# ingonyama-zk/gnark-icicle

Measured on AMD Instinct MI355X. Metric: BN254 G1 MSM Mpoints/s (2^20 points per GPU, sharded MSM), higher is better.
Workload: dtype u32 limbs (BN254 Fp/Fr Montgomery, integer); 1 GPU; BN254 G1 MSM 2^20 random points/scalars per GPU (BASELINE configs[1]); points_per_gpu=1048576, total_points=1048576, parallelism=msm-shard1

## Files before the change

### gnark-icicle_amd/csrc/curve.hpp

```cpp
#pragma once
#include "field.hpp"

namespace gm {

template <class F>
struct FOps;

template <class P>
struct FOps<Fe<P>> {
  using T = Fe<P>;
  GM_DEV static T zero() { return fe_zero<P>(); }
  GM_DEV static T one() { return fe_one<P>(); }
};
template <class P, int B>
struct FOps<Fe2<P, B>> {
  using T = Fe2<P, B>;
  GM_DEV static T zero() { return {fe_zero<P>(), fe_zero<P>()}; }
  GM_DEV static T one() { return {fe_one<P>(), fe_zero<P>()}; }
};

template <class F>
struct Affine {
  F x, y;
};
template <class F>
struct XYZZ {
  F x, y, zz, zzz;
};

template <class F>
GM_DEV bool aff_is_inf(const Affine<F>& p) {
  return fe_is_zero(p.x) && fe_is_zero(p.y);
}

template <class F>
GM_DEV XYZZ<F> xyzz_inf() {
  XYZZ<F> r;
  r.x = FOps<F>::one();
  r.y = FOps<F>::one();
  r.zz = FOps<F>::zero();
  r.zzz = FOps<F>::zero();
  return r;
}
template <class F>
GM_DEV bool xyzz_is_inf(const XYZZ<F>& p) {
  return fe_is_zero(p.zz);
}

template <class F>
GM_DEV XYZZ<F> xyzz_dbl_aff(const Affine<F>& p) {
  F U = fe_dbl(p.y);
  F V = fe_sqr(U);
  F W = fe_mul(U, V);
  F S = fe_mul(p.x, V);
  F X2 = fe_sqr(p.x);
  F M = fe_add(fe_dbl(X2), X2);
  XYZZ<F> r;
  r.x = fe_sub(fe_sqr(M), fe_dbl(S));
  r.y = fe_sub(fe_mul(M, fe_sub(S, r.x)), fe_mul(W, p.y));
  r.zz = V;
  r.zzz = W;
  return r;
}

template <class F>
GM_DEV void xyzz_add_aff(XYZZ<F>& a, const Affine<F>& p) {
  if (aff_is_inf(p)) return;
  if (xyzz_is_inf(a)) {
    a.x = p.x;
    a.y = p.y;
    a.zz = FOps<F>::one();
    a.zzz = FOps<F>::one();
    return;
  }
  F P = fe_sub(fe_mul(p.x, a.zz), a.x);
  F R = fe_sub(fe_mul(p.y, a.zzz), a.y);
  if (fe_is_zero(P)) {
    if (fe_is_zero(R)) {
      a = xyzz_dbl_aff(p);
    } else {
      a = xyzz_inf<F>();
    }
    return;
  }
  F PP = fe_sqr(P);
  F PPP = fe_mul(P, PP);
  a.zz = fe_mul(a.zz, PP);
  F Q = fe_mul(a.x, PP);
  a.zzz = fe_mul(a.zzz, PPP);
  F X3 = fe_sub(fe_sub(fe_sqr(R), PPP), fe_dbl(Q));
  a.y = fe_sub(fe_mul(R, fe_sub(Q, X3)), fe_mul(a.y, PPP));
  a.x = X3;
}

template <class P, int CH = 0>
GM_DEV void xyzz_add_aff_lz(XYZZ<Fe<P>>& a, const Affine<Fe<P>>& p, bool neg) {
  static_assert(P::BITS + 7 <= RADIX * P::N, "lazy reduction needs R' > 128 p");
  using F = Fe<P>;
  if (aff_is_inf(p)) return;
  if (xyzz_is_inf(a)) {
    a.x = p.x;
    a.y = neg ? fe_neg(p.y) : p.y;
    a.zz = fe_one<P>();
    a.zzz = fe_one<P>();
    return;
  }
  F Pd = fe_sub_lz<8>(fe_mul<P, false, CH>(p.x, a.zz), a.x);
  F R = fe_sub_lz<4>(fe_cneg2p_cf(fe_mul<P, false, CH>(p.y, a.zzz), neg), a.y);
  if (fe_is_zero_lz<10>(Pd)) {
    if (fe_is_zero_lz<6>(R)) {
      Affine<F> q = p;
      if (neg) q.y = fe_neg(p.y);
      a = xyzz_dbl_aff(q);
    } else {
      a = xyzz_inf<F>();
    }
    return;
  }
  F PP = fe_sqr<P, false, CH>(Pd);
  F PPP = fe_mul<P, false, CH>(Pd, PP);
  a.zz = fe_mul<P, false, CH>(a.zz, PP);
  F Q = fe_mul<P, false, CH>(a.x, PP);
  a.zzz = fe_mul<P, false, CH>(a.zzz, PPP);
  F X3 = fe_sub2x_lz<6>(fe_sqr<P, false, CH>(R), PPP, Q);
  if constexpr (P::N <= 10)
    a.y = fe_mul2_redc_u<P, CH>(R, fe_sub_cf<9>(Q, X3), fe_negk_cf<5>(a.y), PPP);
  else
    a.y = fe_mul2_redc_u<P, CH>(R, fe_sub_lz<8>(Q, X3), fe_negk_cf<5>(a.y), PPP);
  a.x = X3;
}
template <class P, int BETA>
GM_DEV void xyzz_add_aff_lz(XYZZ<Fe2<P, BETA>>& a, const Affine<Fe2<P, BETA>>& p) {
  static_assert(P::BITS + 7 <= RADIX * P::N, "lazy reduction needs R' > 128 p");
  using F = Fe2<P, BETA>;
  if (aff_is_inf(p)) return;
  if (xyzz_is_inf(a)) {
    a.x = p.x;
    a.y = p.y;
    a.zz = FOps<F>::one();
    a.zzz = FOps<F>::one();
    return;
  }
  F Pd = fe2_sub_lz<2>(fe2_mul_lz(p.x, a.zz), a.x);
  F R = fe2_sub_lz<2>(fe2_mul_lz(p.y, a.zzz), a.y);
  if (fe_is_zero_lz<4>(Pd.a0) && fe_is_zero_lz<4>(Pd.a1)) {
    if (fe_is_zero_lz<4>(R.a0) && fe_is_zero_lz<4>(R.a1)) {
      a = xyzz_dbl_aff(p);
    } else {
      a = xyzz_inf<F>();
    }
    return;
  }
  F PP = fe2_sqr_lz<4>(Pd);
  F PPP = fe2_mul_lz(Pd, PP);
  a.zz = fe2_mul_lz(a.zz, PP);
  F Q = fe2_mul_lz(a.x, PP);
  a.zzz = fe2_mul_lz(a.zzz, PPP);
  F X3 = fe2_sub_lz<4>(fe2_sub_lz<2>(fe2_sqr_lz<4>(R), PPP), fe2_add_lz(Q, Q));
  fe2_to2p<8>(X3);
  F Y3 = fe2_sub_lz<2>(fe2_mul_lz(R, fe2_sub_lz<2>(Q, X3)), fe2_mul_lz(a.y, PPP));
  fe2_to2p<4>(Y3);
  a.x = X3;
  a.y = Y3;
}
template <class P, int BETA>
GM_DEV XYZZ<Fe2<P, BETA>> xyzz_canon_lz(const XYZZ<Fe2<P, BETA>>& a) {
  auto c = [](const Fe2<P, BETA>& v) { return Fe2<P, BETA>{fe_canon<1>(v.a0), fe_canon<1>(v.a1)}; };
  return {c(a.x), c(a.y), c(a.zz), c(a.zzz)};
}

template <class P>
GM_DEV XYZZ<Fe<P>> xyzz_canon_lz(const XYZZ<Fe<P>>& a) {
  XYZZ<Fe<P>> r;
  r.x = fe_canon<3>(a.x);
  r.y = fe_canon<2>(a.y);
  r.zz = fe_canon<1>(a.zz);
  r.zzz = fe_canon<1>(a.zzz);
  return r;
}

template <class F>
GM_DEV XYZZ<F> xyzz_dbl(const XYZZ<F>& a) {
  F U = fe_dbl(a.y);
  F V = fe_sqr(U);
  F W = fe_mul(U, V);
  F S = fe_mul(a.x, V);
  F X2 = fe_sqr(a.x);
  F M = fe_add(fe_dbl(X2), X2);
  XYZZ<F> r;
  r.x = fe_sub(fe_sqr(M), fe_dbl(S));
  r.y = fe_sub(fe_mul(M, fe_sub(S, r.x)), fe_mul(W, a.y));
  r.zz = fe_mul(V, a.zz);
  r.zzz = fe_mul(W, a.zzz);
  return r;
}

template <class F>
GM_DEV XYZZ<F> xyzz_add(const XYZZ<F>& a, const XYZZ<F>& b) {
  if (xyzz_is_inf(a)) return b;
  if (xyzz_is_inf(b)) return a;
  F U1 = fe_mul(a.x, b.zz);
  F U2 = fe_mul(b.x, a.zz);
  F S1 = fe_mul(a.y, b.zzz);
  F S2 = fe_mul(b.y, a.zzz);
  F P = fe_sub(U2, U1);
  F R = fe_sub(S2, S1);
  if (fe_is_zero(P)) {
    if (fe_is_zero(R)) return xyzz_dbl(a);
    return xyzz_inf<F>();
  }
  F PP = fe_sqr(P);
  F PPP = fe_mul(P, PP);
  F Q = fe_mul(U1, PP);
  XYZZ<F> r;
  r.x = fe_sub(fe_sub(fe_sqr(R), PPP), fe_dbl(Q));
  r.y = fe_sub(fe_mul(R, fe_sub(Q, r.x)), fe_mul(S1, PPP));
  r.zz = fe_mul(fe_mul(a.zz, b.zz), PP);
  r.zzz = fe_mul(fe_mul(a.zzz, b.zzz), PPP);
  return r;
}

template <class P>
GM_DEV XYZZ<Fe<P>> xyzz_canon2(const XYZZ<Fe<P>>& a) {
  return {fe_canon<1>(a.x), fe_canon<1>(a.y), fe_canon<1>(a.zz), fe_canon<1>(a.zzz)};
}

template <class P>
GM_DEV XYZZ<Fe<P>> xyzz_add_lz(const XYZZ<Fe<P>>& a, const XYZZ<Fe<P>>& b) {
  using F = Fe<P>;
  if (xyzz_is_inf(a)) return b;
  if (xyzz_is_inf(b)) return a;
  const F U1 = fe_mul_lz(a.x, b.zz);
  const F U2 = fe_mul_lz(b.x, a.zz);
  const F S1 = fe_mul_lz(a.y, b.zzz);
  const F S2 = fe_mul_lz(b.y, a.zzz);
  const F Pd = fe_sub_lz<2>(U2, U1);
  const F R = fe_sub_lz<2>(S2, S1);
  if (fe_is_zero_lz<4>(Pd)) {
    if (fe_is_zero_lz<4>(R)) return xyzz_dbl(xyzz_canon2(a));
    return xyzz_inf<F>();
  }
  const F PP = fe_sqr_lz(Pd);
  const F PPP = fe_mul_lz(Pd, PP);
  const F Q = fe_mul_lz(U1, PP);
  F X3 = fe_sub_lz<4>(fe_sub_lz<2>(fe_sqr_lz(R), PPP), fe_add_lz(Q, Q));
  fe_to2p<8>(X3);
  const F Y3 = fe_mul2_redc_u(R, fe_sub_lz<2>(Q, X3), fe_negk_cf<3>(S1), PPP);
  XYZZ<F> r;
  r.x = X3;
  r.y = Y3;
  r.zz = fe_mul_lz(fe_mul_lz(a.zz, b.zz), PP);
  r.zzz = fe_mul_lz(fe_mul_lz(a.zzz, b.zzz), PPP);
  return r;
}

template <class F>
GM_DEV Affine<F> load_affine_gnark(const uint32_t* __restrict__ src) {
  Affine<F> r;
  r.x = Coord<F>::load_internal(src);
  r.y = Coord<F>::load_internal(src + Coord<F>::WORDS);
  return r;
}
template <class F>
GM_DEV Affine<F> load_affine_packed(const uint32_t* __restrict__ src) {
  Affine<F> r;
  r.x = Coord<F>::load_packed(src);
  r.y = Coord<F>::load_packed(src + Coord<F>::WORDS);
  return r;
}
template <class F>
GM_DEV void store_affine_packed(uint32_t* __restrict__ dst, const Affine<F>& a) {
  Coord<F>::store_packed(dst, a.x);
  Coord<F>::store_packed(dst + Coord<F>::WORDS, a.y);
}
template <class F>
GM_DEV void store_affine_gnark(uint32_t* __restrict__ dst, const Affine<F>& a) {
  Coord<F>::store_gnark(dst, a.x);
  Coord<F>::store_gnark(dst + Coord<F>::WORDS, a.y);
}

template <class F>
GM_DEV Affine<F> aff_neg(const Affine<F>& p) {
  Affine<F> r;
  r.x = p.x;
  r.y = fe_neg(p.y);
  return r;
}

template <class F>
GM_DEV XYZZ<F> xyzz_mul_small(const XYZZ<F>& a, uint32_t k) {
  XYZZ<F> r = xyzz_inf<F>();
  if (k == 0) return r;
  int top = 31 - __builtin_clz(k);
  r = a;
  for (int b = top - 1; b >= 0; b--) {
    r = xyzz_dbl(r);
    if ((k >> b) & 1) r = xyzz_add(r, a);
  }
  return r;
}

using Bn254Fp2 = Fe2<Bn254Fp, -1>;
using Bls377Fp2 = Fe2<Bls377Fp, -5>;

}
```

### gnark-icicle_amd/csrc/field.hpp

```cpp
#pragma once
#include <hip/hip_runtime.h>
#include <cstdint>
#include "field_constants.hpp"

namespace gm {

#define GM_DEV __device__ __forceinline__
#define GM_HD __host__ __device__ __forceinline__

constexpr int RADIX = 29;
constexpr uint32_t LIMB_MASK = (1u << RADIX) - 1;

#define GM_CONST_ARRAY_FN(FN, N, INIT)       \
  GM_HD static constexpr uint32_t FN(int i) { \
    constexpr uint32_t a[N] = INIT;           \
    return a[i];                              \
  }

#define GM_DEFINE_FIELD(NAME, TAG)                                              \
  struct NAME {                                                                 \
    static constexpr int N = GM_##TAG##_N29;              \
    static constexpr int NG = GM_##TAG##_NG;               \
    static constexpr int BITS = GM_##TAG##_BITS;                                \
    static constexpr uint32_t INV = GM_##TAG##_INV29;                           \
// ... 225 lines not shown
    for (int i = (k - N + 1 > 0 ? k - N + 1 : 0); i <= (k - 1 < N - 1 ? k - 1 : N - 1); i++) {
      acc += (uint64_t)m[i] * P::p(k - i);
      GM_STRICT_STEP(acc, CHAIN);
    }
    if (k < N) {
      m[k] = ((uint32_t)acc * P::INV) & LIMB_MASK;
      acc += (uint64_t)m[k] * P::p(0);
    } else {
      r.v[k - N] = (uint32_t)acc & LIMB_MASK;
    }
    acc >>= RADIX;
  }
  r.v[N - 1] = (uint32_t)acc;
  if constexpr (REDUCE) fe_reduce_once(r);
  return r;
}

template <class P, bool REDUCE = true, int CHAIN = GM_FE_CHAIN>
GM_DEV Fe<P> fe_sqr(const Fe<P>& a) {
  constexpr int N = P::N;
  uint32_t m[N];
  Fe<P> r;
  uint64_t acc = 0;
#pragma unroll
  for (int k = 0; k < 2 * N - 1; k++) {
    if constexpr (CHAIN) {
      if (k) __asm__ volatile("" : "+v"(acc));
    }
    if constexpr (CHAIN >= 2) {
#pragma unroll
      for (int i = (k - N + 1 > 0 ? k - N + 1 : 0); i <= (k < N - 1 ? k : N - 1); i++) {
        const int j = k - i;
        if (i < j) {
          acc += (uint64_t)a.v[i] * (a.v[j] << 1);
          GM_STRICT_STEP(acc, CHAIN);
        }
      }
    } else {
      uint64_t cross = 0;
#pragma unroll
      for (int i = (k - N + 1 > 0 ? k - N + 1 : 0); i <= (k < N - 1 ? k : N - 1); i++) {
        const int j = k - i;
        if (i < j) cross += (uint64_t)a.v[i] * a.v[j];
      }
      acc += cross << 1;
    }
    if ((k & 1) == 0) {
      acc += (uint64_t)a.v[k / 2] * a.v[k / 2];
      GM_STRICT_STEP(acc, CHAIN);
    }
#pragma unroll
    for (int i = (k - N + 1 > 0 ? k - N + 1 : 0); i <= (k - 1 < N - 1 ? k - 1 : N - 1); i++) {
      acc += (uint64_t)m[i] * P::p(k - i);
      GM_STRICT_STEP(acc, CHAIN);
    }
    if (k < N) {
      m[k] = ((uint32_t)acc * P::INV) & LIMB_MASK;
      acc += (uint64_t)m[k] * P::p(0);
    } else {
      r.v[k - N] = (uint32_t)acc & LIMB_MASK;
    }
    acc >>= RADIX;
  }
  r.v[N - 1] = (uint32_t)acc;
  if constexpr (REDUCE) fe_reduce_once(r);
  return r;
}

template <class P, int K>
GM_HD constexpr uint32_t kp_limb(int i) {
  uint64_t carry = 0;
  for (int j = 0; j < P::N; j++) {
    const uint64_t v = (uint64_t)P::p(j) * K + carry;
    if (j == i) return j == P::N - 1 ? (uint32_t)v : (uint32_t)(v & LIMB_MASK);
    carry = v >> RADIX;
  }
  return 0;
}
template <class P>
GM_HD constexpr uint32_t kp_top(int j) {
  uint64_t carry = 0, v = 0;
  for (int i = 0; i < P::N; i++) {
    v = (uint64_t)P::p(i) * (uint64_t)j + carry;
    carry = v >> RADIX;
  }
  return (uint32_t)v;
}
template <class P>
GM_DEV Fe<P> fe_mul_lz(const Fe<P>& a, const Fe<P>& b) { return fe_mul<P, false>(a, b); }
template <class P>
GM_DEV Fe<P> fe_mul_lz_chain(const Fe<P>& a, const Fe<P>& b) { return fe_mul<P, false, true>(a, b); }
template <class P>
GM_DEV Fe<P> fe_sqr_lz(const Fe<P>& a) { return fe_sqr<P, false>(a); }
template <class P, int CHAIN = GM_FE_CHAIN>
GM_DEV Fe<P> fe_mul2_redc_u(const Fe<P>& x1, const Fe<P>& y1, const Fe<P>& x2, const Fe<P>& y2) {
  constexpr int N = P::N;
  static_assert(N <= 14, "unsigned two-product column bound");
  uint32_t m[N];
  Fe<P> r;
  uint64_t acc = 0;
#pragma unroll
  for (int k = 0; k < 2 * N - 1; k++) {
    if constexpr (CHAIN) {
      if (k) __asm__ volatile("" : "+v"(acc));
    }
#pragma unroll
    for (int i = (k - N + 1 > 0 ? k - N + 1 : 0); i <= (k < N - 1 ? k : N - 1); i++) {
      acc += (uint64_t)x1.v[i] * y1.v[k - i];
      GM_STRICT_STEP(acc, CHAIN);
      acc += (uint64_t)x2.v[i] * y2.v[k - i];
      GM_STRICT_STEP(acc, CHAIN);
    }
#pragma unroll
    for (int i = (k - N + 1 > 0 ? k - N + 1 : 0); i <= (k - 1 < N - 1 ? k - 1 : N - 1); i++) {
      acc += (uint64_t)m[i] * P::p(k - i);
      GM_STRICT_STEP(acc, CHAIN);
    }
    if (k < N) {
      m[k] = ((uint32_t)acc * P::INV) & LIMB_MASK;
      acc += (uint64_t)m[k] * P::p(0);
    } else {
      r.v[k - N] = (uint32_t)acc & LIMB_MASK;
    }
    acc >>= RADIX;
  }
  r.v[N - 1] = (uint32_t)acc;
  return r;
}

template <class P>
GM_DEV Fe<P> fe_add_lz(const Fe<P>& a, const Fe<P>& b) {
  Fe<P> r;
  uint32_t c = 0;
#pragma unroll
  for (int i = 0; i < P::N; i++) {
    const uint32_t s = a.v[i] + b.v[i] + c;
    r.v[i] = i == P::N - 1 ? s : (s & LIMB_MASK);
    c = s >> RADIX;
  }
  return r;
}
template <int K, class P>
GM_DEV Fe<P> fe_sub_lz(const Fe<P>& a, const Fe<P>& b) {
  Fe<P> r;
  int32_t c = 0;
#pragma unroll
  for (int i = 0; i < P::N; i++) {
    const int32_t d = (int32_t)(a.v[i] + kp_limb<P, K>(i)) - (int32_t)b.v[i] + c;
    c = d >> RADIX;
    r.v[i] = i == P::N - 1 ? (uint32_t)d : ((uint32_t)d & LIMB_MASK);
  }
  return r;
}
template <int K, class P>
GM_DEV void fe_reduce_k(Fe<P>& a) {
  Fe<P> t;
  int32_t borrow = 0;
#pragma unroll
  for (int i = 0; i < P::N; i++) {
    const int32_t d = (int32_t)a.v[i] - (int32_t)kp_limb<P, K>(i) + borrow;
    borrow = d >> RADIX;
    t.v[i] = (uint32_t)d & LIMB_MASK;
  }
  const bool ge = borrow == 0;
#pragma unroll
  for (int i = 0; i < P::N; i++) a.v[i] = ge ? t.v[i] : a.v[i];
}
template <class P>
GM_HD constexpr uint32_t p2_borrowed_limb(int i) {
  return i == 0 ? kp_limb<P, 2>(0) + (1u << RADIX)
                : (i == P::N - 1 ? kp_limb<P, 2>(i) - 1u : kp_limb<P, 2>(i) + (1u << RADIX) - 1u);
}
template <class P, int K>
GM_HD constexpr uint32_t kp_borrowed_limb(int i) {
  return i == 0 ? kp_limb<P, K>(0) + (1u << RADIX)
                : (i == P::N - 1 ? kp_limb<P, K>(i) - 1u : kp_limb<P, K>(i) + (1u << RADIX) - 1u);
}
template <int K, class P>
GM_DEV Fe<P> fe_negk_cf(const Fe<P>& s) {
  Fe<P> r;
#pragma unroll
  for (int i = 0; i < P::N; i++) r.v[i] = kp_borrowed_limb<P, K>(i) - s.v[i];
  return r;
}
template <int K, class P>
GM_DEV Fe<P> fe_sub_cf(const Fe<P>& a, const Fe<P>& b) {
  static_assert(P::N <= 11, "unnormalised product operand column bound");
  Fe<P> r;
#pragma unroll
  for (int i = 0; i < P::N; i++) r.v[i] = a.v[i] + (kp_borrowed_limb<P, K>(i) - b.v[i]);
  return r;
}
template <class P>
GM_DEV Fe<P> fe_cneg2p_cf(const Fe<P>& s, bool neg) {
  Fe<P> r;
#pragma unroll
  for (int i = 0; i < P::N; i++) r.v[i] = neg ? p2_borrowed_limb<P>(i) - s.v[i] : s.v[i];
  return r;
}
template <int K, class P>
GM_DEV Fe<P> fe_sub2x_lz(const Fe<P>& a, const Fe<P>& b, const Fe<P>& c) {
  Fe<P> r;
  int32_t cy = 0;
#pragma unroll
  for (int i = 0; i < P::N; i++) {
    const int32_t d = (int32_t)(a.v[i] + kp_limb<P, K>(i)) - (int32_t)(b.v[i] + (c.v[i] << 1)) + cy;
    cy = d >> RADIX;
    r.v[i] = i == P::N - 1 ? (uint32_t)d : ((uint32_t)d & LIMB_MASK);
  }
  return r;
}
template <int L, class P>
GM_DEV Fe<P> fe_canon(Fe<P> a) {
  if constexpr (L >= 4) fe_reduce_k<8>(a);
  if constexpr (L >= 3) fe_reduce_k<4>(a);
  if constexpr (L >= 2) fe_reduce_k<2>(a);
  if constexpr (L >= 1) fe_reduce_k<1>(a);
  return a;
}
template <int K, class P>
GM_DEV bool fe_is_zero_lz(const Fe<P>& a) {
  static_assert(K <= 16, "fe_canon<4> covers a < 16p");
  const uint32_t top = a.v[P::N - 1];
  bool hit = false;
#pragma unroll
  for (int j = 0; j < K; j++) hit |= top == kp_top<P>(j);
  if (!hit) return false;
  return fe_is_zero(fe_canon<4>(a));
}

template <class P>
GM_DEV Fe<P> fe_to_internal(const Fe<P>& gnark_form) { return fe_mul(gnark_form, GM_FE_CONST(P, kin)); }
template <class P>
GM_DEV Fe<P> fe_to_gnark(const Fe<P>& internal) { return fe_mul(internal, GM_FE_CONST(P, kout)); }
template <class P>
GM_DEV Fe<P> fe_gnark_to_canonical(const Fe<P>& gnark_form) { return fe_mul(gnark_form, GM_FE_CONST(P, kcan)); }
template <class P>
GM_DEV Fe<P> fe_canonical_to_gnark(const Fe<P>& x) { return fe_mul(x, GM_FE_CONST(P, kgn)); }
template <class P>
GM_DEV Fe<P> fe_to_mont(const Fe<P>& x) { return fe_mul(x, GM_FE_CONST(P, r2)); }
template <class P>
GM_DEV Fe<P> fe_from_mont(const Fe<P>& internal) {
  Fe<P> o = fe_zero<P>();
  o.v[0] = 1;
  return fe_mul(internal, o);
}

template <class P>
GM_DEV Fe<P> fe_inv(const Fe<P>& a) {
  Fe<P> r = fe_one<P>();
  for (int i = P::NG - 1; i >= 0; i--) {
    const uint32_t e = P::pm2(i);
    for (int b = 31; b >= 0; b--) {
      r = fe_sqr(r);
      if ((e >> b) & 1) r = fe_mul(r, a);
    }
  }
  return r;
}

template <class P, int BETA>
struct Fe2 {
  using Base = P;
  Fe<P> a0, a1;
};

template <class P, int BETA>
GM_DEV Fe2<P, BETA> fe_add(const Fe2<P, BETA>& a, const Fe2<P, BETA>& b) {
  return {fe_add(a.a0, b.a0), fe_add(a.a1, b.a1)};
}
template <class P, int BETA>
GM_DEV Fe2<P, BETA> fe_sub(const Fe2<P, BETA>& a, const Fe2<P, BETA>& b) {
  return {fe_sub(a.a0, b.a0), fe_sub(a.a1, b.a1)};
}
template <class P, int BETA>
GM_DEV Fe2<P, BETA> fe_dbl(const Fe2<P, BETA>& a) {
  return {fe_dbl(a.a0), fe_dbl(a.a1)};
}
template <class P, int BETA>
GM_DEV Fe2<P, BETA> fe_neg(const Fe2<P, BETA>& a) {
  return {fe_neg(a.a0), fe_neg(a.a1)};
}
template <class P, int BETA>
GM_DEV bool fe_is_zero(const Fe2<P, BETA>& a) {
  return fe_is_zero(a.a0) && fe_is_zero(a.a1);
}
template <class P, int BETA>
GM_DEV Fe<P> mul_by_beta(const Fe<P>& x) {
  static_assert(BETA == -1 || BETA == -5, "unsupported non-residue");
  if constexpr (BETA == -1) {
    return fe_neg(x);
  } else {
    Fe<P> x2 = fe_dbl(x);
    Fe<P> x4 = fe_dbl(x2);
    return fe_neg(fe_add(x4, x));
  }
}
template <class P, int BETA>
GM_DEV Fe2<P, BETA> fe_mul(const Fe2<P, BETA>& a, const Fe2<P, BETA>& b) {
  Fe<P> v0 = fe_mul(a.a0, b.a0);
  Fe<P> v1 = fe_mul(a.a1, b.a1);
  Fe<P> s = fe_mul(fe_add(a.a0, a.a1), fe_add(b.a0, b.a1));
  Fe2<P, BETA> r;
  r.a0 = fe_add(v0, mul_by_beta<P, BETA>(v1));
  r.a1 = fe_sub(fe_sub(s, v0), v1);
  return r;
// ... 116 lines not shown
```

### gnark-icicle_amd/csrc/msm_impl.hpp

```cpp
#pragma once
#include "curves.hpp"
#include "msm.hpp"
#include "pair_fp2.hpp"
#include "runtime.hpp"

#include <hip/hip_ext.h>

#include <cmath>
#include <cstdlib>
#include <cstring>
#include <type_traits>

namespace gm {

template <class Fr>
GM_DEV uint32_t window_bits(const FeG<Fr>& k, uint32_t bit, uint32_t mask) {
  const uint32_t idx = bit >> 5, sh = bit & 31;
  uint32_t lo = 0, hi = 0;
#pragma unroll
  for (int i = 0; i < Fr::NG; i++) {
    lo = (idx == (uint32_t)i) ? k.w[i] : lo;
    hi = (idx + 1 == (uint32_t)i) ? k.w[i] : hi;
  }
  const uint64_t v = ((uint64_t)hi << 32) | lo;
// ... 192 lines not shown
  static constexpr bool ok = true;
  using U = unsigned __int128;
  GM_DEV static void split(const uint64_t (&k64)[4], U& k1, U& k2, uint32_t& neg2) {
    U q = glv_mulshift<5>(k64, GlvBls377::g);
    const U lam = ((U)GlvBls377::LAM_HI << 64) | GlvBls377::LAM_LO;
    const U klo = ((U)k64[1] << 64) | k64[0];
    U r = klo - q * lam;
    if (r >= lam) {
      r -= lam;
      q += 1;
    }
    k1 = r;
    k2 = q;
    neg2 = 0;
  }
};

template <class C>
__global__ void __launch_bounds__(1024) k_msm_digits_glv(const uint32_t* __restrict__ scalars, DigitGeom g,
                                                         uint32_t n0, uint32_t NC, uint32_t* __restrict__ dig,
                                                         uint32_t* __restrict__ ccount) {
  using Fr = typename C::Fr;
  extern __shared__ uint32_t dg_lds[];
  const uint32_t t = threadIdx.x;
  for (uint32_t q = t; q < NC; q += DG_THREADS) dg_lds[q] = 0;
  __syncthreads();
  const uint32_t base = blockIdx.x * DG_THREADS * DG_PPT;
  for (uint32_t r = 0; r < DG_PPT; r++) {
    const uint32_t i = base + r * DG_THREADS + t;
    if (i >= n0) break;
    const FeG<Fr> k = load_scalar_canonical<Fr>(scalars, i);
    uint64_t k64[4];
#pragma unroll
    for (int j = 0; j < 4; j++) k64[j] = (uint64_t)k.w[2 * j] | ((uint64_t)k.w[2 * j + 1] << 32);
    unsigned __int128 k1, k2;
    uint32_t neg2;
    Glv<C>::split(k64, k1, k2, neg2);
    FeG<Fr> m1, m2;
#pragma unroll
    for (int j = 0; j < Fr::NG; j++) {
      m1.w[j] = j < 4 ? (uint32_t)(k1 >> (32 * j)) : 0u;
      m2.w[j] = j < 4 ? (uint32_t)(k2 >> (32 * j)) : 0u;
    }
    emit_digits<Fr>(m1, 0u, i, g, dig, dg_lds);
    emit_digits<Fr>(m2, neg2, n0 + i, g, dig, dg_lds);
  }
  __syncthreads();
  for (uint32_t q = t; q < NC; q += DG_THREADS)
    if (dg_lds[q]) atomicAdd(&ccount[q], dg_lds[q]);
}

template <class F, bool GLV>
__global__ void __launch_bounds__(256) k_msm_convert_points_lds(const uint32_t* __restrict__ src, size_t n,
                                                                uint32_t* __restrict__ dst) {
  constexpr int PW = 2 * Coord<F>::WORDS;
  constexpr uint32_t Q = PW / 4;
  static_assert(PW % 4 == 0, "points are whole uint4s");
  __shared__ uint4 tile[256 * (Q + 1)];
  const size_t b0 = (size_t)blockIdx.x * 256;
  const uint32_t np = (uint32_t)min((size_t)256, n - b0);
  const uint32_t t = threadIdx.x;
  const uint4* s = reinterpret_cast<const uint4*>(src) + b0 * Q;
  for (uint32_t q = t; q < np * Q; q += 256) tile[(q / Q) * (Q + 1) + q % Q] = s[q];
  __syncthreads();
  uint32_t* mine = reinterpret_cast<uint32_t*>(tile + t * (Q + 1));
  Affine<F> a;
  if (t < np) {
    a = load_affine_gnark<F>(mine);
    store_affine_packed<F>(mine, a);
  }
  __syncthreads();
  uint4* d = reinterpret_cast<uint4*>(dst) + b0 * Q;
  for (uint32_t q = t; q < np * Q; q += 256) d[q] = tile[(q / Q) * (Q + 1) + q % Q];
  if constexpr (GLV) {
    __syncthreads();
    if (t < np) {
      a.x = glv_phi_x(a.x);
      store_affine_packed<F>(mine, a);
    }
    __syncthreads();
    uint4* d2 = reinterpret_cast<uint4*>(dst) + (n + b0) * Q;
    for (uint32_t q = t; q < np * Q; q += 256) d2[q] = tile[(q / Q) * (Q + 1) + q % Q];
  }
}

template <class F>
__global__ void __launch_bounds__(256) k_msm_convert_points(const uint32_t* __restrict__ src, size_t n,
                                                            uint32_t* __restrict__ dst) {
  const size_t i = (size_t)blockIdx.x * blockDim.x + threadIdx.x;
  if (i >= n) return;
  constexpr int PW = 2 * Coord<F>::WORDS;
  store_affine_packed<F>(dst + i * PW, load_affine_gnark<F>(src + i * PW));
}

template <class F>
__global__ void __launch_bounds__(128) k_msm_precompute(uint32_t* __restrict__ pts, size_t n, size_t stride,
                                                        uint32_t c, uint32_t W, uint32_t wn) {
  const size_t i = (size_t)blockIdx.x * blockDim.x + threadIdx.x;
  if (i >= n) return;
  constexpr int PW = 2 * Coord<F>::WORDS;
  const Affine<F> P = load_affine_packed<F>(pts + i * PW);
  Affine<F> zero;
  zero.x = FOps<F>::zero();
  zero.y = FOps<F>::zero();
  if (aff_is_inf(P)) {
    for (uint32_t w = 1; w < W; w++) store_affine_packed<F>(pts + (w * stride + i) * PW, zero);
    return;
  }
  XYZZ<F> acc;
  acc.x = P.x;
  acc.y = P.y;
  acc.zz = FOps<F>::one();
  acc.zzz = FOps<F>::one();
  for (uint32_t w = 1; w < W; w++) {
    const uint32_t cw = (w - 1 >= wn) ? c - 1 : c;
    for (uint32_t k = 0; k < cw; k++) acc = xyzz_dbl(acc);
    Affine<F> r = zero;
    if (!xyzz_is_inf(acc)) {
      const F t = fe_inv(fe_mul(acc.zz, acc.zzz));
      r.x = fe_mul(acc.x, fe_mul(t, acc.zzz));
      r.y = fe_mul(acc.y, fe_mul(t, acc.zz));
    }
    store_affine_packed<F>(pts + (w * stride + i) * PW, r);
  }
}

template <int PW>
struct PackedPt {
  uint32_t w[PW];
};
template <int PW>
GM_DEV PackedPt<PW> load_packed_pt(const uint32_t* __restrict__ src) {
  static_assert(PW % 4 == 0, "packed points are whole 16-byte chunks");
  PackedPt<PW> r;
#pragma unroll
  for (int q = 0; q < PW / 4; q++) {
    const uint4 v = reinterpret_cast<const uint4*>(src)[q];
    r.w[4 * q] = v.x;
    r.w[4 * q + 1] = v.y;
    r.w[4 * q + 2] = v.z;
    r.w[4 * q + 3] = v.w;
  }
  return r;
}

template <class F>
struct LazyAcc {
  static constexpr bool on = false;
  template <bool CH = false>
  GM_DEV static void add(XYZZ<F>& a, Affine<F> p, bool neg) {
    if (neg) p.y = fe_neg(p.y);
    xyzz_add_aff(a, p);
  }
  GM_DEV static XYZZ<F> canon(const XYZZ<F>& a) { return a; }
};
template <class P>
struct LazyAcc<Fe<P>> {
  static constexpr bool on = true;
  template <bool CH = false>
  GM_DEV static void add(XYZZ<Fe<P>>& a, const Affine<Fe<P>>& p, bool neg) {
    xyzz_add_aff_lz<P, CH ? 2 : 0>(a, p, neg);
  }
  GM_DEV static XYZZ<Fe<P>> canon(const XYZZ<Fe<P>>& a) { return xyzz_canon_lz(a); }
};
template <class P, int B>
struct LazyAcc<Fe2<P, B>> {
  static constexpr bool on = true;
  template <bool CH = false>
  GM_DEV static void add(XYZZ<Fe2<P, B>>& a, Affine<Fe2<P, B>> p, bool neg) {
    if (neg) p.y = fe_neg(p.y);
    xyzz_add_aff_lz(a, p);
  }
  GM_DEV static XYZZ<Fe2<P, B>> canon(const XYZZ<Fe2<P, B>>& a) { return xyzz_canon_lz(a); }
};

template <class F>
GM_DEV void accum_emit(uint32_t b, const XYZZ<F>& acc_raw, bool is_first, bool is_last, uint32_t start,
                       uint32_t end, uint32_t t, const uint32_t* __restrict__ offsets,
                       XYZZ<F>* __restrict__ buckets, XYZZ<F>* __restrict__ part_first,
                       XYZZ<F>* __restrict__ part_last) {
  const XYZZ<F> acc = LazyAcc<F>::canon(acc_raw);
  const uint32_t bs = offsets[b], be = offsets[b + 1];
  if (bs >= start && be <= end) {
    buckets[b] = acc;
  } else {
    if (is_first) part_first[t] = acc;
    if (is_last) part_last[t] = acc;
  }
}

GM_DEV void wave_stamp_begin(unsigned long long* stamp) {
  if (stamp && blockIdx.x < 64 && (threadIdx.x & 63) == 0)
    atomicMin(stamp + blockIdx.x * 32, (unsigned long long)wall_clock64());
}
GM_DEV void wave_stamp_end(unsigned long long* stamp) {
  if (stamp && (threadIdx.x & 63) == 0)
    atomicMax(stamp + (blockIdx.x & 63) * 32 + 1, (unsigned long long)wall_clock64());
}

template <class F, bool CH, bool PREFETCH = false>
GM_DEV void accum_seg_body_v4(const uint32_t* __restrict__ points, uint32_t n, const uint32_t* __restrict__ keys,
                              const uint32_t* __restrict__ vals, const uint32_t* __restrict__ offsets,
                              uint32_t total, uint32_t K, XYZZ<F>* __restrict__ buckets,
                              XYZZ<F>* __restrict__ part_first, XYZZ<F>* __restrict__ part_last,
                              uint32_t* __restrict__ err) {
  const uint32_t t = blockIdx.x * blockDim.x + threadIdx.x;
  const uint32_t Mv = offsets[total];
  const uint32_t start = t * K;
  if (start >= Mv) return;
  const uint32_t end = min(start + K, Mv);
  uint4 kg = *reinterpret_cast<const uint4*>(keys + start);
  uint4 vg = *reinterpret_cast<const uint4*>(vals + start);
  bool first = true;
  XYZZ<F> acc = xyzz_inf<F>();
  uint32_t cur = kg.x;
  uint32_t v = vg.x;
  if ((v & 0x7fffffffu) >= n) {
    atomicOr(err, 2u);
    return;
  }
  constexpr int PW = 2 * Coord<F>::WORDS;
  PackedPt<PW> P;
  if (PREFETCH) P = load_packed_pt<PW>(points + (size_t)(v & 0x7fffffffu) * PW);
  for (uint32_t q = start; q < end; q++) {
    const uint32_t k = kg.x;
    if (((q - start) & 3) == 3) {
      if (q + 1 < end) {
        kg = *reinterpret_cast<const uint4*>(keys + q + 1);
        vg = *reinterpret_cast<const uint4*>(vals + q + 1);
      }
    } else {
      kg = make_uint4(kg.y, kg.z, kg.w, kg.w);
      vg = make_uint4(vg.y, vg.z, vg.w, vg.w);
    }
    const uint32_t vn = vg.x;
    PackedPt<PW> Pn;
    if (q + 1 < end) {
      if ((vn & 0x7fffffffu) >= n) {
        atomicOr(err, 2u);
        return;
      }
      if (PREFETCH) Pn = load_packed_pt<PW>(points + (size_t)(vn & 0x7fffffffu) * PW);
    }
    if (!PREFETCH) P = load_packed_pt<PW>(points + (size_t)(v & 0x7fffffffu) * PW);
    if (k != cur) {
      accum_emit(cur, acc, first, false, start, end, t, offsets, buckets, part_first, part_last);
      first = false;
      acc = xyzz_inf<F>();
      cur = k;
    }
    const Affine<F> A = load_affine_packed<F>(P.w);
    LazyAcc<F>::template add<CH>(acc, A, (v >> 31) != 0);
    v = vn;
    if (PREFETCH) P = Pn;
  }
  accum_emit(cur, acc, first, true, start, end, t, offsets, buckets, part_first, part_last);
}

template <class F>
__global__ void __launch_bounds__(128) __attribute__((amdgpu_waves_per_eu(4)))
k_msm_accum_seg_ch(const uint32_t* __restrict__ points, uint32_t n, const uint32_t* __restrict__ keys,
                   const uint32_t* __restrict__ vals, const uint32_t* __restrict__ offsets, uint32_t total,
                   uint32_t K, XYZZ<F>* __restrict__ buckets, XYZZ<F>* __restrict__ part_first,
                   XYZZ<F>* __restrict__ part_last, uint32_t* __restrict__ err,
                   unsigned long long* __restrict__ stamp) {
  wave_stamp_begin(stamp);
  accum_seg_body_v4<F, true>(points, n, keys, vals, offsets, total, K, buckets, part_first, part_last, err);
  wave_stamp_end(stamp);
}
template <class F>
struct AccumW4 {
  static constexpr bool ok = false;
};
template <class P>
struct AccumW4<Fe<P>> {
  static constexpr bool ok = P::N <= 9;
};
template <class F>
__global__ void __launch_bounds__(128) k_msm_accum_seg_pf4(const uint32_t* __restrict__ points, uint32_t n,
                                                           const uint32_t* __restrict__ keys,
                                                           const uint32_t* __restrict__ vals,
                                                           const uint32_t* __restrict__ offsets, uint32_t total,
                                                           uint32_t K, XYZZ<F>* __restrict__ buckets,
                                                           XYZZ<F>* __restrict__ part_first,
                                                           XYZZ<F>* __restrict__ part_last,
                                                           uint32_t* __restrict__ err,
                                                           unsigned long long* __restrict__ stamp) {
  wave_stamp_begin(stamp);
  accum_seg_body_v4<F, false, true>(points, n, keys, vals, offsets, total, K, buckets, part_first, part_last, err);
  wave_stamp_end(stamp);
}
template <class F>
constexpr auto g1_accum_kernel() {
  if constexpr (AccumW4<F>::ok) return k_msm_accum_seg_ch<F>;
  else return k_msm_accum_seg_pf4<F>;
}

template <class F>
struct PairSel {
  static constexpr bool ok = false;
};
template <class P, int B>
struct PairSel<Fe2<P, B>> {
  static constexpr bool ok = true;
  static constexpr auto kernel() {
    if constexpr (P::N <= 9) return k_msm_accum_seg_pair<P, B, false, 3, true, true>;
    else return k_msm_accum_seg_pair<P, B, false, GM_PAIR_WPE, true>;
  }
  static constexpr auto fixup() { return k_msm_fixup_pair<P, B>; }
  static constexpr auto fixup_edge() { return k_msm_fixup_edge_pair<P, B>; }
  static constexpr auto fix_tree() { return k_msm_fix_tree_pair<P, B>; }
  static constexpr auto fixup_long() { return k_msm_fixup_long_pair<P, B>; }
  static constexpr auto seg() { return k_msm_seg_pair<P, B>; }
  static constexpr auto bitsum() { return k_msm_bitsum_pair<P, B>; }
};
template <class F>
constexpr bool kOneLane = !PairSel<F>::ok;

template <class F>
struct FullAdd {
  GM_DEV static XYZZ<F> add(const XYZZ<F>& a, const XYZZ<F>& b) { return xyzz_add(a, b); }
  GM_DEV static XYZZ<F> canon(const XYZZ<F>& a) { return a; }
};
template <class P>
struct FullAdd<Fe<P>> {
  GM_DEV static XYZZ<Fe<P>> add(const XYZZ<Fe<P>>& a, const XYZZ<Fe<P>>& b) { return xyzz_add_lz(a, b); }
  GM_DEV static XYZZ<Fe<P>> canon(const XYZZ<Fe<P>>& a) { return xyzz_canon2(a); }
};

constexpr uint32_t FIX_SERIAL = 8;

template <class F>
__global__ void __launch_bounds__(128) k_msm_fixup(const uint32_t* __restrict__ offsets, uint32_t total,
                                                   uint32_t K, XYZZ<F>* __restrict__ buckets,
                                                   const XYZZ<F>* __restrict__ part_first,
                                                   const XYZZ<F>* __restrict__ part_last,
                                                   uint32_t* __restrict__ maxspan) {
  const uint32_t b = blockIdx.x * blockDim.x + threadIdx.x;
  if (b >= total) return;
  const uint32_t bs = offsets[b], be = offsets[b + 1];
  if (be == bs) return;
  const uint32_t t0 = bs / K, t1 = (be - 1) / K;
  if (t0 == t1) return;
  if (t1 - t0 > FIX_SERIAL) {
    atomicMax(maxspan, t1 - t0);
    return;
  }
  XYZZ<F> acc = part_last[t0];
  for (uint32_t t = t0 + 1; t <= t1; t++) acc = FullAdd<F>::add(acc, part_first[t]);
  buckets[b] = FullAdd<F>::canon(acc);
}

template <class F>
__global__ void __launch_bounds__(128) k_msm_fixup_edge(const uint32_t* __restrict__ keys,
                                                        const uint32_t* __restrict__ offsets, uint32_t total,
                                                        uint32_t K, uint32_t nslices,
                                                        XYZZ<F>* __restrict__ buckets,
                                                        const XYZZ<F>* __restrict__ part_first,
                                                        const XYZZ<F>* __restrict__ part_last,
                                                        uint32_t* __restrict__ maxspan) {
  const uint32_t t = blockIdx.x * blockDim.x + threadIdx.x + 1;
  if (t >= nslices) return;
  const size_t q = (size_t)t * K;
  if (q >= offsets[total]) return;
  const uint32_t b = keys[q];
  const uint32_t bs = offsets[b];
  if (bs >= q || bs / K != t - 1) return;
  const uint32_t t0 = t - 1, t1 = (offsets[b + 1] - 1) / K;
  if (t1 - t0 > FIX_SERIAL) {
    atomicMax(maxspan, t1 - t0);
    return;
  }
  XYZZ<F> acc = part_last[t0];
  for (uint32_t u = t; u <= t1; u++) acc = FullAdd<F>::add(acc, part_first[u]);
  buckets[b] = FullAdd<F>::canon(acc);
}
template <class F>
__global__ void __launch_bounds__(128) k_msm_fix_tree(const uint32_t* __restrict__ keys,
                                                      const uint32_t* __restrict__ offsets, uint32_t total,
                                                      uint32_t K, uint32_t nslices, uint32_t d,
                                                      XYZZ<F>* __restrict__ part_first) {
  const uint32_t t = blockIdx.x * blockDim.x + threadIdx.x;
  if (t >= nslices || (size_t)t * K >= offsets[total]) return;
  const uint32_t b = keys[(size_t)t * K];
  const uint32_t t0 = offsets[b] / K, t1 = (offsets[b + 1] - 1) / K;
  if (t1 - t0 <= FIX_SERIAL || t <= t0) return;
  const uint32_t rel = t - (t0 + 1), len = t1 - t0, step = 1u << d;
  if ((rel & ((step << 1) - 1)) == 0 && rel + step < len)
    part_first[t] = FullAdd<F>::canon(FullAdd<F>::add(part_first[t], part_first[t + step]));
}

template <class F>
__global__ void __launch_bounds__(128) k_msm_fixup_long(const uint32_t* __restrict__ offsets, uint32_t total,
                                                        uint32_t K, XYZZ<F>* __restrict__ buckets,
                                                        const XYZZ<F>* __restrict__ part_first,
                                                        const XYZZ<F>* __restrict__ part_last) {
  const uint32_t b = blockIdx.x * blockDim.x + threadIdx.x;
  if (b >= total) return;
  const uint32_t bs = offsets[b], be = offsets[b + 1];
  if (be == bs) return;
  const uint32_t t0 = bs / K, t1 = (be - 1) / K;
  if (t1 - t0 <= FIX_SERIAL) return;
  buckets[b] = FullAdd<F>::canon(FullAdd<F>::add(part_last[t0], part_first[t0 + 1]));
}

constexpr uint32_t BS_THREADS = 256;
template <class F>
__global__ void __launch_bounds__(128) k_msm_seg(const XYZZ<F>* __restrict__ buckets,
                                                 const uint32_t* __restrict__ offsets, uint32_t nb, uint32_t L,
                                                 uint32_t nseg, uint32_t W, XYZZ<F>* __restrict__ nodes) {
  const uint32_t t = blockIdx.x * blockDim.x + threadIdx.x;
  if (t >= W * nseg) return;
  const uint32_t w = t / nseg, s = t % nseg;
  const size_t b0 = (size_t)w * nb + (size_t)s * L;
  const XYZZ<F>* B = buckets + b0;
  const uint32_t* O = offsets + b0;
  uint32_t o_hi = O[L];
  uint32_t o_lo = O[L - 1];
  XYZZ<F> S = o_lo == o_hi ? xyzz_inf<F>() : B[L - 1], T = S;
  for (int j = (int)L - 2; j >= 0; j--) {
    o_hi = o_lo;
    o_lo = O[j];
    S = FullAdd<F>::add(S, o_lo == o_hi ? xyzz_inf<F>() : B[j]);
    T = FullAdd<F>::add(T, S);
  }
  nodes[2 * (size_t)t] = FullAdd<F>::canon(S);
  nodes[2 * (size_t)t + 1] = FullAdd<F>::canon(T);
}

template <class F>
__global__ void __launch_bounds__(BS_THREADS) k_msm_bitsum(const XYZZ<F>* __restrict__ in, uint32_t m,
                                                    uint32_t Qin, uint32_t NT, uint32_t lgNT,
                                                    XYZZ<F>* __restrict__ out) {
  extern __shared__ __attribute__((aligned(16))) char smem_raw[];
  XYZZ<F>* X = reinterpret_cast<XYZZ<F>*>(smem_raw);
  const uint32_t groups = m / NT;
  const uint32_t w = blockIdx.x / groups, j = blockIdx.x % groups;
  const XYZZ<F>* src = in + ((size_t)w * m + (size_t)j * NT) * Qin;
  for (uint32_t q = threadIdx.x; q < NT * Qin; q += blockDim.x) X[q] = src[q];
  __syncthreads();
  for (uint32_t d = 0; d < lgNT; d++) {
    const uint32_t qc = Qin + d + 1;
    const uint32_t tasks = (NT >> (d + 1)) * qc;
    const uint32_t child = (Qin << d);
    XYZZ<F> r0, r1;
    uint32_t s0 = 0xffffffffu, s1 = 0xffffffffu;
    {
      const uint32_t t = threadIdx.x;
      if (t < tasks) {
        const uint32_t p = t / qc, q = t % qc, base = p * 2 * child;
        r0 = (q + 1 < qc) ? FullAdd<F>::canon(FullAdd<F>::add(X[base + q], X[base + child + q])) : X[base + child];
        s0 = base + q;
      }
    }
    {
      const uint32_t t = threadIdx.x + blockDim.x;
      if (t < tasks) {
        const uint32_t p = t / qc, q = t % qc, base = p * 2 * child;
        r1 = (q + 1 < qc) ? FullAdd<F>::canon(FullAdd<F>::add(X[base + q], X[base + child + q])) : X[base + child];
        s1 = base + q;
      }
    }
    __syncthreads();
    if (s0 != 0xffffffffu) X[s0] = r0;
    if (s1 != 0xffffffffu) X[s1] = r1;
    __syncthreads();
  }
  const uint32_t Qout = Qin + lgNT;
  XYZZ<F>* dst = out + ((size_t)w * groups + j) * Qout;
  for (uint32_t q = threadIdx.x; q < Qout; q += blockDim.x) dst[q] = X[q];
}

template <class F>
__global__ void __launch_bounds__(128) k_msm_export(const XYZZ<F>* __restrict__ nodes, uint32_t count,
                                                    uint32_t* __restrict__ out) {
  const uint32_t t = blockIdx.x * blockDim.x + threadIdx.x;
  if (t >= count) return;
  uint32_t* o = out + (size_t)t * 4 * Coord<F>::WORDS;
  const XYZZ<F> r = nodes[t];
  Coord<F>::store_gnark(o, r.x);
  Coord<F>::store_gnark(o + Coord<F>::WORDS, r.y);
  Coord<F>::store_gnark(o + 2 * Coord<F>::WORDS, r.zz);
  Coord<F>::store_gnark(o + 3 * Coord<F>::WORDS, r.zzz);
}

static int choose_window(size_t n, int bits) {
  int best = 8;
  double best_cost = 1e300;
  for (int c = 8; c <= 20; c++) {
    const double W = (double)((bits + 1 + c - 1) / c);
    const double cost = (double)n * W + 3.0 * W * (double)(1u << (c - 1));
    if (cost < best_cost) {
      best_cost = cost;
      best = c;
    }
  }
  return best;
}

template <class C>
int msm_plan(gm_ctx* ctx, Arena& arena, const void* scalars_dev, size_t n, const MsmPrecomp* pre,
             MsmPlan& plan, bool glv) {
  hipStream_t st = ctx->stream;
  plan = MsmPlan();
  plan.n = n;
  plan.bits = C::FR_BITS;
  if (n == 0) return GM_OK;
  if (glv && (!Glv<C>::ok || (pre && pre->c))) {
    set_error("msm: the GLV split needs a plain (not precomputed) layout");
    return GM_ERR_INVALID;
  }
  const size_t n0 = n;
  if (glv) {
    n = 2 * n0;
    plan.n = n;
    plan.bits = 127;
  }
  if (n >= (size_t(1) << 31)) {
    set_error("msm: n must be < 2^31");
    return GM_ERR_INVALID;
  }
  const bool shared = pre && pre->c;
  if (shared && (pre->stride < n || (size_t)pre->W * pre->stride >= (size_t(1) << 31) || pre->narrow >= pre->W ||
                 (size_t)pre->c * pre->W - pre->narrow < (size_t)C::FR_BITS + 1)) {
    set_error("msm: precomputed point set does not cover this MSM");
    return GM_ERR_INVALID;
  }
  const uint32_t c = shared ? pre->c
                            : (ctx->msm_c_override ? (uint32_t)ctx->msm_c_override
                                                   : (uint32_t)choose_window(n, plan.bits));
  const uint32_t W = shared ? pre->W : (uint32_t)(plan.bits + 1 + c - 1) / c;
  plan.c = c;
  plan.W = W;
  plan.nb = 1u << (c - 1);
  plan.Wred = shared ? 1 : W;
  plan.total = plan.Wred * plan.nb;
  plan.npts = shared ? (size_t)W * pre->stride : n;
  const size_t M = (size_t)W * n;
  plan.M = M;
  if (M >= (size_t(1) << 31)) {
    set_error("msm: n * windows must be < 2^31");
    return GM_ERR_INVALID;
  }
  SortGeom sg;
  sg.T = plan.total;
  sg.M = M;
  sg.F = 4;
  const double bin_entries = glv || shared ? 4096.0 : 2048.0;
  while (sg.F < 13 && (double)M * std::ldexp(1.0, (int)sg.F + 1) <= bin_entries * sg.T) sg.F++;
  auto bins = [&](uint32_t sh) { return (uint32_t)(((uint64_t)sg.T + (1ull << sh) - 1) >> sh); };
  auto touched = [&](uint32_t sh) { return shared ? bins(sh) : std::max(1u, plan.nb >> sh); };
  const char* ming = getenv("GM_MSM_SORT_MING");
  sg.G = ming ? (uint32_t)std::min(10, std::max(0, atoi(ming))) : 0u;
  const uint32_t max_touched = (shared && M < (size_t(1) << 24)) ? 8192u : 512u;
  while (sg.G < 10 && (touched(sg.F + sg.G) > max_touched || bins(sg.F + sg.G) > 8192)) sg.G++;
  while (sg.G && sg.F + sg.G > 31) sg.G--;
  sg.NC = bins(sg.F);
  sg.NS = bins(sg.F + sg.G);
  if (sg.NS > 8192) {
    set_error("msm: too many buckets for the sort");
    return GM_ERR_INVALID;
  }
  int rc;
  DevBuf dig, keys_out, vals_out, offsets, scount;
  if ((rc = dig.alloc(arena, sizeof(uint32_t) * M)) || (rc = keys_out.alloc(arena, sizeof(uint32_t) * M)) ||
      (rc = vals_out.alloc(arena, sizeof(uint32_t) * M)) ||
      (rc = offsets.alloc(arena, sizeof(uint32_t) * ((size_t)plan.total + 1))) ||
      (rc = scount.alloc(arena, sizeof(uint32_t) * sg.NS)))
    return rc;
  DigitGeom g;
  g.n = (uint32_t)n;
  g.c = c;
  g.W = W;
  g.nb = plan.nb;
  g.shared_stride = shared ? (uint32_t)pre->stride : 0u;
  g.wn = shared ? W - pre->narrow : W;
  if (!shared && !glv) {
    const uint32_t narrow = c * W - (uint32_t)(plan.bits + 1);
    if (narrow < W) g.wn = W - narrow;
  }
  plan.wn = g.wn;
  g.F = sg.F + sg.G;
  {
    ProfScope ps(ctx, "msm_digits");
    GM_HIP(hipMemsetAsync(scount.p, 0, sizeof(uint32_t) * sg.NS, st));
    if constexpr (Glv<C>::ok) {
      if (glv)
        hipLaunchKernelGGL(k_msm_digits_glv<C>, dim3(blocks_for(n0, DG_THREADS * DG_PPT)), dim3(DG_THREADS),
                         sizeof(uint32_t) * sg.NS, st, reinterpret_cast<const uint32_t*>(scalars_dev), g,
                           (uint32_t)n0, sg.NS, dig.as<uint32_t>(), scount.as<uint32_t>());
    }
    if (!glv)
      hipLaunchKernelGGL(k_msm_digits<typename C::Fr>, dim3(blocks_for(n, DG_THREADS * DG_PPT)), dim3(DG_THREADS),
                         sizeof(uint32_t) * sg.NS, st, reinterpret_cast<const uint32_t*>(scalars_dev), g, sg.NS,
                         dig.as<uint32_t>(), scount.as<uint32_t>());
    GM_HIP(hipGetLastError());
  }
  {
    ProfScope ps(ctx, "msm_sort");
    if ((rc = msm_sort_digits(ctx, arena, sg, n, W, plan.nb, g.shared_stride, dig.as<uint32_t>(),
                              scount.as<uint32_t>(), keys_out.as<uint32_t>(), vals_out.as<uint32_t>(),
                              offsets.as<uint32_t>())))
      return rc;
  }
  plan.keys = keys_out.as<uint32_t>();
  plan.vals = vals_out.as<uint32_t>();
  plan.offsets = offsets.as<uint32_t>();
  return GM_OK;
}

template <class C, bool G2>
int msm_reduce(gm_ctx* ctx, MsmTail& t) {
// ... 367 lines not shown
```

Before: 685.5 Mpoints/s.

## Skip canonicalization of lazy bucket accumulators and simplify accumulate emit

Bucket accumulators are now stored in their lazily reduced form instead of being canonicalized after each bucket, and the fixup and tree kernels likewise skip canonicalization, relying on xyzz_add_lz tolerating wider input ranges. The emit logic replaces accum_emit's offsets loads and range checks with a precomputed continuation flag and next-key lookup. Negation of the first point uses a cheaper p-minus subtraction. This removes per-bucket reduction work and global offset reads, but risks overflow or incorrect equality checks if the lazy bounds assumed downstream do not hold.

Result: faster. 708.9 Mpoints/s (median of 6 runs) (+3.4%).

```diff
diff --git a/gnark-icicle_amd/csrc/curve.hpp b/gnark-icicle_amd/csrc/curve.hpp
--- a/gnark-icicle_amd/csrc/curve.hpp
+++ b/gnark-icicle_amd/csrc/curve.hpp
@@ -100,7 +100,7 @@
   if (aff_is_inf(p)) return;
   if (xyzz_is_inf(a)) {
     a.x = p.x;
-    a.y = neg ? fe_neg(p.y) : p.y;
+    a.y = neg ? fe_pminus(p.y) : p.y;
     a.zz = fe_one<P>();
     a.zzz = fe_one<P>();
     return;
@@ -167,16 +167,6 @@
 GM_DEV XYZZ<Fe2<P, BETA>> xyzz_canon_lz(const XYZZ<Fe2<P, BETA>>& a) {
   auto c = [](const Fe2<P, BETA>& v) { return Fe2<P, BETA>{fe_canon<1>(v.a0), fe_canon<1>(v.a1)}; };
   return {c(a.x), c(a.y), c(a.zz), c(a.zzz)};
-}
-
-template <class P>
-GM_DEV XYZZ<Fe<P>> xyzz_canon_lz(const XYZZ<Fe<P>>& a) {
-  XYZZ<Fe<P>> r;
-  r.x = fe_canon<3>(a.x);
-  r.y = fe_canon<2>(a.y);
-  r.zz = fe_canon<1>(a.zz);
-  r.zzz = fe_canon<1>(a.zzz);
-  return r;
 }
 
 template <class F>
@@ -224,6 +214,10 @@
 GM_DEV XYZZ<Fe<P>> xyzz_canon2(const XYZZ<Fe<P>>& a) {
   return {fe_canon<1>(a.x), fe_canon<1>(a.y), fe_canon<1>(a.zz), fe_canon<1>(a.zzz)};
 }
+template <class P>
+GM_DEV XYZZ<Fe<P>> xyzz_canon_raw(const XYZZ<Fe<P>>& a) {
+  return {fe_canon<3>(a.x), fe_canon<1>(a.y), fe_canon<1>(a.zz), fe_canon<1>(a.zzz)};
+}
 
 template <class P>
 GM_DEV XYZZ<Fe<P>> xyzz_add_lz(const XYZZ<Fe<P>>& a, const XYZZ<Fe<P>>& b) {
@@ -237,7 +231,7 @@
   const F Pd = fe_sub_lz<2>(U2, U1);
   const F R = fe_sub_lz<2>(S2, S1);
   if (fe_is_zero_lz<4>(Pd)) {
-    if (fe_is_zero_lz<4>(R)) return xyzz_dbl(xyzz_canon2(a));
+    if (fe_is_zero_lz<4>(R)) return xyzz_dbl(xyzz_canon_raw(a));
     return xyzz_inf<F>();
   }
   const F PP = fe_sqr_lz(Pd);
diff --git a/gnark-icicle_amd/csrc/field.hpp b/gnark-icicle_amd/csrc/field.hpp
--- a/gnark-icicle_amd/csrc/field.hpp
+++ b/gnark-icicle_amd/csrc/field.hpp
@@ -401,6 +401,18 @@
   }
   return r;
 }
+template <class P>
+GM_DEV Fe<P> fe_pminus(const Fe<P>& a) {
+  Fe<P> r;
+  int32_t borrow = 0;
+#pragma unroll
+  for (int i = 0; i < P::N; i++) {
+    const int32_t d = (int32_t)P::p(i) - (int32_t)a.v[i] + borrow;
+    borrow = d >> RADIX;
+    r.v[i] = i == P::N - 1 ? (uint32_t)d : ((uint32_t)d & LIMB_MASK);
+  }
+  return r;
+}
 template <int K, class P>
 GM_DEV void fe_reduce_k(Fe<P>& a) {
   Fe<P> t;
diff --git a/gnark-icicle_amd/csrc/msm_impl.hpp b/gnark-icicle_amd/csrc/msm_impl.hpp
--- a/gnark-icicle_amd/csrc/msm_impl.hpp
+++ b/gnark-icicle_amd/csrc/msm_impl.hpp
@@ -368,7 +368,6 @@
     if (neg) p.y = fe_neg(p.y);
     xyzz_add_aff(a, p);
   }
-  GM_DEV static XYZZ<F> canon(const XYZZ<F>& a) { return a; }
 };
 template <class P>
 struct LazyAcc<Fe<P>> {
@@ -377,33 +376,7 @@
   GM_DEV static void add(XYZZ<Fe<P>>& a, const Affine<Fe<P>>& p, bool neg) {
     xyzz_add_aff_lz<P, CH ? 2 : 0>(a, p, neg);
   }
-  GM_DEV static XYZZ<Fe<P>> canon(const XYZZ<Fe<P>>& a) { return xyzz_canon_lz(a); }
-};
-template <class P, int B>
-struct LazyAcc<Fe2<P, B>> {
-  static constexpr bool on = true;
-  template <bool CH = false>
-  GM_DEV static void add(XYZZ<Fe2<P, B>>& a, Affine<Fe2<P, B>> p, bool neg) {
-    if (neg) p.y = fe_neg(p.y);
-    xyzz_add_aff_lz(a, p);
-  }
-  GM_DEV static XYZZ<Fe2<P, B>> canon(const XYZZ<Fe2<P, B>>& a) { return xyzz_canon_lz(a); }
-};
-
-template <class F>
-GM_DEV void accum_emit(uint32_t b, const XYZZ<F>& acc_raw, bool is_first, bool is_last, uint32_t start,
-                       uint32_t end, uint32_t t, const uint32_t* __restrict__ offsets,
-                       XYZZ<F>* __restrict__ buckets, XYZZ<F>* __restrict__ part_first,
-                       XYZZ<F>* __restrict__ part_last) {
-  const XYZZ<F> acc = LazyAcc<F>::canon(acc_raw);
-  const uint32_t bs = offsets[b], be = offsets[b + 1];
-  if (bs >= start && be <= end) {
-    buckets[b] = acc;
-  } else {
-    if (is_first) part_first[t] = acc;
-    if (is_last) part_last[t] = acc;
-  }
-}
+};
 
 GM_DEV void wave_stamp_begin(unsigned long long* stamp) {
   if (stamp && blockIdx.x < 64 && (threadIdx.x & 63) == 0)
@@ -427,9 +400,10 @@
   const uint32_t end = min(start + K, Mv);
   uint4 kg = *reinterpret_cast<const uint4*>(keys + start);
   uint4 vg = *reinterpret_cast<const uint4*>(vals + start);
-  bool first = true;
   XYZZ<F> acc = xyzz_inf<F>();
   uint32_t cur = kg.x;
+  bool cont_prev = start > 0 && keys[start - 1] == cur;
+  const uint32_t key_after = end < Mv ? keys[end] : 0xffffffffu;
   uint32_t v = vg.x;
   if ((v & 0x7fffffffu) >= n) {
     atomicOr(err, 2u);
@@ -460,8 +434,8 @@
     }
     if (!PREFETCH) P = load_packed_pt<PW>(points + (size_t)(v & 0x7fffffffu) * PW);
     if (k != cur) {
-      accum_emit(cur, acc, first, false, start, end, t, offsets, buckets, part_first, part_last);
-      first = false;
+      *(cont_prev ? part_first + t : buckets + cur) = acc;
+      cont_prev = false;
       acc = xyzz_inf<F>();
       cur = k;
     }
@@ -470,7 +444,7 @@
     v = vn;
     if (PREFETCH) P = Pn;
   }
-  accum_emit(cur, acc, first, true, start, end, t, offsets, buckets, part_first, part_last);
+  *(cont_prev ? part_first + t : (key_after == cur ? part_last + t : buckets + cur)) = acc;
 }
 
 template <class F>
@@ -537,11 +511,13 @@
 struct FullAdd {
   GM_DEV static XYZZ<F> add(const XYZZ<F>& a, const XYZZ<F>& b) { return xyzz_add(a, b); }
   GM_DEV static XYZZ<F> canon(const XYZZ<F>& a) { return a; }
+  GM_DEV static XYZZ<F> canon2(const XYZZ<F>& a) { return a; }
 };
 template <class P>
 struct FullAdd<Fe<P>> {
   GM_DEV static XYZZ<Fe<P>> add(const XYZZ<Fe<P>>& a, const XYZZ<Fe<P>>& b) { return xyzz_add_lz(a, b); }
-  GM_DEV static XYZZ<Fe<P>> canon(const XYZZ<Fe<P>>& a) { return xyzz_canon2(a); }
+  GM_DEV static XYZZ<Fe<P>> canon(const XYZZ<Fe<P>>& a) { return xyzz_canon_raw(a); }
+  GM_DEV static XYZZ<Fe<P>> canon2(const XYZZ<Fe<P>>& a) { return xyzz_canon2(a); }
 };
 
 constexpr uint32_t FIX_SERIAL = 8;
@@ -564,7 +540,7 @@
   }
   XYZZ<F> acc = part_last[t0];
   for (uint32_t t = t0 + 1; t <= t1; t++) acc = FullAdd<F>::add(acc, part_first[t]);
-  buckets[b] = FullAdd<F>::canon(acc);
+  buckets[b] = acc;
 }
 
 template <class F>
@@ -589,7 +565,7 @@
   }
   XYZZ<F> acc = part_last[t0];
   for (uint32_t u = t; u <= t1; u++) acc = FullAdd<F>::add(acc, part_first[u]);
-  buckets[b] = FullAdd<F>::canon(acc);
+  buckets[b] = acc;
 }
 template <class F>
 __global__ void __launch_bounds__(128) k_msm_fix_tree(const uint32_t* __restrict__ keys,
@@ -603,7 +579,7 @@
   if (t1 - t0 <= FIX_SERIAL || t <= t0) return;
   const uint32_t rel = t - (t0 + 1), len = t1 - t0, step = 1u << d;
   if ((rel & ((step << 1) - 1)) == 0 && rel + step < len)
-    part_first[t] = FullAdd<F>::canon(FullAdd<F>::add(part_first[t], part_first[t + step]));
+    part_first[t] = FullAdd<F>::add(part_first[t], part_first[t + step]);
 }
 
 template <class F>
@@ -617,7 +593,7 @@
   if (be == bs) return;
   const uint32_t t0 = bs / K, t1 = (be - 1) / K;
   if (t1 - t0 <= FIX_SERIAL) return;
-  buckets[b] = FullAdd<F>::canon(FullAdd<F>::add(part_last[t0], part_first[t0 + 1]));
+  buckets[b] = FullAdd<F>::add(part_last[t0], part_first[t0 + 1]);
 }
 
 constexpr uint32_t BS_THREADS = 256;
@@ -665,7 +641,7 @@
       const uint32_t t = threadIdx.x;
       if (t < tasks) {
         const uint32_t p = t / qc, q = t % qc, base = p * 2 * child;
-        r0 = (q + 1 < qc) ? FullAdd<F>::canon(FullAdd<F>::add(X[base + q], X[base + child + q])) : X[base + child];
+        r0 = (q + 1 < qc) ? FullAdd<F>::canon2(FullAdd<F>::add(X[base + q], X[base + child + q])) : X[base + child];
         s0 = base + q;
       }
     }
@@ -673,7 +649,7 @@
       const uint32_t t = threadIdx.x + blockDim.x;
       if (t < tasks) {
         const uint32_t p = t / qc, q = t % qc, base = p * 2 * child;
-        r1 = (q + 1 < qc) ? FullAdd<F>::canon(FullAdd<F>::add(X[base + q], X[base + child + q])) : X[base + child];
+        r1 = (q + 1 < qc) ? FullAdd<F>::canon2(FullAdd<F>::add(X[base + q], X[base + child + q])) : X[base + child];
         s1 = base + q;
       }
     }
```
